# CliMA/ClimaOcean.jl

Measured on AMD Instinct MI355X. Metric: flux-kernel surface cells/s (update_state!: JRA55 interp + similarity-theory fluxes + net fluxes), higher is better.
Workload: dtype f64

## Files before the change

climaocean.jl_amd/csrc/coflux_abi.cpp:

```cpp
#include "coflux_ctx.hpp"

static thread_local std::string g_error;
static RcclApi g_rccl;

int cf_fail(cf_ctx* ctx, int code, const char* fmt, ...) {
    char buf[1024];
    va_list ap;
    va_start(ap, fmt);
    vsnprintf(buf, sizeof buf, fmt, ap);
    va_end(ap);
    g_error = buf;
    if (ctx) {
        std::lock_guard<std::mutex> lock(ctx->error_mutex);
        ctx->error = buf;
    }
    return code;
}

static int wait_for_halos(cf_ctx* ctx);
int cf_flush_deferred_prefetch(cf_ctx* ctx);

static bool roughness_ok(const cf_roughness& r, bool scalar) {
    if (scalar) {
        if (r.kind == CF_SCALAR_ROUGHNESS_CONSTANT) return r.constant_length > 0;
// ... 795 lines not shown
    if (ctx->deferred.valid && ctx->deferred.out.u == atmos->u) CHECK(cf_flush_deferred_prefetch(ctx));
    for (auto& p : ctx->prefetch) {
        if (!p.valid || p.key != atmos->u) continue;
        if (!p.on_main) HIP_TRY(ctx, hipStreamWaitEvent(ctx->stream, p.done, 0));
        prefetched = p.level1 == src->level1 && p.level2 == src->level2 && p.tf == src->time_fraction;
        p.valid = false;
    }
    const bool fuse = net_fluxes_fused(ctx);
    if (!prefetched) HIP_TRY(ctx, launch_interpolate(ctx->stream, ctx->launch, ctx->grid, src, w, atmos));
    if (rec) HIP_TRY(ctx, hipEventRecord(ev[1], ctx->stream));
    CHECK(wait_for_halos(ctx));
    const bool tail_lean = ctx->launch.d_lean_info && ctx->fast.specialization == SOLVER_OCEAN_LEAN && ctx->launch.solver == CF_SOLVER_TABLES;
    const bool tail_ly = ctx->fast.specialization == SOLVER_LY && ctx->launch.solver == CF_SOLVER_TABLES;
    const bool tail = fuse && !hold_tail_work && ctx->merged_prefetch == 2 && ctx->deferred.valid &&
                      interp_tile_fits(ctx, 40960) && ctx->deferred.out.u != atmos->u && (tail_lean || tail_ly);
    const bool ride = hold_tail_work && ocean_rider && fuse && tail_lean && !rec;
    HaloRider halo_rider{};
    const HaloRider* halo = nullptr;
    if (ctx->halo_request.valid) {
        ctx->halo_request.valid = false;
        if (tail && tail_lean && !ride && ctx->d_halo_counters && lean_halo_rides(ctx->launch, ctx->fast)) {
            HaloRider& H = halo_rider;
            H.M = ctx->peer;
            H.F = ctx->halo_request.F;
            H.counters = ctx->d_halo_counters;
            H.seq = ++ctx->peer_seq;
            ++ctx->halo_in_launch_count;
            for (int dir = 0; dir < 2; ++dir)
                if ((dir == 0 ? ctx->peer.south : ctx->peer.north) != nullptr) {
                    ctx->halo_expect_sent[dir] += (unsigned long long)H.F.n;
                    ctx->halo_expect_done[dir] += (unsigned long long)H.F.n;
                }
            for (int dir = 0; dir < 2; ++dir) {
                H.expect_sent[dir] = ctx->halo_expect_sent[dir];
                H.expect_done[dir] = ctx->halo_expect_done[dir];
            }
            H.status = ctx->d_peer_status;
            H.rows = ctx->halo_request.rows;
            H.blocks = 2 * H.F.n;
            H.chunk_south = ctx->launch.chunk_south;
            H.chunk_north = ctx->launch.chunk_north;
            H.wait_south = ctx->peer.south != nullptr;
            H.wait_north = ctx->peer.north != nullptr;
            halo = &halo_rider;
        } else {
            CHECK(cf_peer_halo_launch_now(ctx, &ctx->halo_request.F, ctx->halo_request.rows));
        }
    }
    if (ride) {
        HIP_TRY(ctx, make_ocean_rider(ctx->launch, ctx->dev, ctx->fast, ctx->grid, ocean, atmos, fluxes, ice, net, ctx->d_land_freshwater,
                                      ocean_rider));
    } else if (tail) {
        int rows = 4, blocks = 1;
        interpolate_grid(ctx->launch, ctx->grid, &rows, &blocks);
        static const int tail_cap = [] {
            const char* e = experiment_knob("COFLUX_TAIL_BLOCKS");
            return e ? std::max(1, std::atoi(e)) : 0;
        }();
        if (tail_cap > 0) blocks = std::min(blocks, tail_cap);
        static const int tail_pos = [] {
            const char* e = experiment_knob("COFLUX_TAIL_POS");
            return e ? std::atoi(e) : -1;
        }();
        if (tail_lean)
            HIP_TRY(ctx, launch_ao_fluxes_lean(ctx->stream, ctx->launch, ctx->dev, ctx->fast, ctx->grid, ocean, atmos, fluxes, ice, net,
                                               ctx->d_land_freshwater, &ctx->deferred.src, &ctx->deferred.w, &ctx->deferred.out, rows, blocks, tail_pos, halo));
        else
            HIP_TRY(ctx, launch_ly_fluxes_with_tail(ctx->stream, ctx->launch, ctx->dev, ctx->fast, ctx->grid, ocean, atmos, fluxes, ice, net,
                                                    ctx->d_land_freshwater, &ctx->deferred.src, &ctx->deferred.w, &ctx->deferred.out, rows, blocks));
        CHECK(deferred_went_out_on_main(ctx));
    } else
    HIP_TRY(ctx, launch_ao_fluxes(ctx->stream, ctx->launch, ctx->dev, ctx->fast, ctx->grid, ocean, atmos, fluxes,
                                  fuse ? ice : nullptr, fuse ? net : nullptr, ctx->d_land_freshwater));
    const bool merge = fuse && !hold_tail_work && ctx->merged_prefetch == 1 && ctx->deferred.valid && interp_tile_fits(ctx, 65536) &&
                       ctx->deferred.out.u != atmos->u;
    if (ctx->merged_prefetch == 0) CHECK(cf_flush_deferred_prefetch(ctx));
    if (rec) HIP_TRY(ctx, hipEventRecord(ev[2], ctx->stream));
    if (merge) {
        HIP_TRY(ctx, launch_interpolate_and_stress(ctx->stream, ctx->launch, ctx->dev, ctx->grid, &ctx->deferred.src, &ctx->deferred.w,
                                                   &ctx->deferred.out, ocean, fluxes, ice, net));
        CHECK(deferred_went_out_on_main(ctx));
    } else if (fuse && hold_tail_work) {
        if (stress_held) *stress_held = true;
    } else if (fuse)
        HIP_TRY(ctx, launch_net_stress(ctx->stream, ctx->dev, ctx->grid, ocean, fluxes, ice, net));
    else
        HIP_TRY(ctx, launch_net_fluxes(ctx->stream, ctx->dev, ctx->grid, ocean, atmos, fluxes, ice, w, net, ctx->d_land_freshwater));
    if (rec) {
        HIP_TRY(ctx, hipEventRecord(ev[3], ctx->stream));
        ++ctx->prof_count;
    }
    if (!hold_tail_work && ctx->merged_prefetch != 0 && ctx->deferred.valid && ctx->deferred.out.u != atmos->u) {
        HIP_TRY(ctx, launch_interpolate(ctx->stream, ctx->launch, ctx->grid, &ctx->deferred.src, &ctx->deferred.w, &ctx->deferred.out));
        CHECK(deferred_went_out_on_main(ctx));
    }
    return CF_OK;
}

int cf_update_state(cf_ctx* ctx, const cf_atmos_source* src, const cf_interp_weights* w,
                    const cf_ocean_surface* ocean, const cf_exchange_fields* atmos,
                    const cf_interface_fluxes* fluxes, const cf_sea_ice_fields* ice, const cf_net_ocean_fluxes* net) {
    return update_state_impl(ctx, src, w, ocean, atmos, fluxes, ice, net, false, nullptr);
}

int cf_profile_enable(cf_ctx* ctx, int max_records) {
    if (!ctx || max_records < 0) return fail(ctx, CF_ERR_INVALID, "cf_profile_enable: bad arguments");
    for (hipEvent_t e : ctx->prof_events) (void)hipEventDestroy(e);
// ... 513 lines not shown
```

climaocean.jl_amd/csrc/coflux_interp.hip:

```cpp
#include <hip/hip_runtime.h>

#include <algorithm>
#include <cstdlib>

#include "coflux_interp_cell.hpp"
#include "coflux_interp_tiles.hpp"
#include "coflux_kernel_types.hpp"
#include "coflux_kernels.h"

namespace coflux {

template <int ROWS>
__global__ __launch_bounds__(64 * IT_WAVES) void interpolate_kernel(SourceDesc S, WeightDesc Wt, GridDesc G,
                                                                     Exchange E, int cap) {
    interpolate_tiles<ROWS>(S, Wt, G, E, cap, (int)blockIdx.x, (int)gridDim.x);
}

struct StressArgs {
    const void* mask;
    const double* rtx;
    const double* rty;
    IceIn I;
    double* tau_x;
    double* tau_y;
// ... 86 lines not shown
    const int i = idx - jj * wx - G.ring, j = jj - G.ring;
    const size_t k = cell_index(G, i, j);
    const double fi = Wt.separable ? Wt.fi[i + G.hx] : Wt.fi[k];
    const double fj = Wt.separable ? Wt.fj[j + G.hy] : Wt.fj[k];
    const double xi = fi - floor(fi), eta = fj - floor(fj);
    const int i0 = (int)trunc(fi), ja = (int)trunc(fj);
    const int is0 = wrap_index(i0, ns_x), is1 = wrap_index(i0 + (fi > 0.0 ? 1 : (fi < 0.0 ? -1 : 0)), ns_x);
    const int j0 = min(max(ja, 0), ns_y - 1), j1 = min(max(ja + (fj > 0.0 ? 1 : (fj < 0.0 ? -1 : 0)), 0), ns_y - 1);
    const size_t g00 = (size_t)j0 * ns_x + is0, g10 = (size_t)j0 * ns_x + is1, g01 = (size_t)j1 * ns_x + is0, g11 = (size_t)j1 * ns_x + is1;
    const size_t plane = (size_t)ns_x * ns_y;
    const double w00 = (1.0 - xi) * (1.0 - eta), w01 = (1.0 - xi) * eta, w10 = xi * (1.0 - eta), w11 = xi * eta;
    auto value = [&](const float* d) {
        const float* a = d + (size_t)level1 * plane;
        const float* b = d + (size_t)level2 * plane;
        return bilinear(w00, w01, w10, w11, blend_levels(a[g00], b[g00], tf), blend_levels(a[g01], b[g01], tf),
                        blend_levels(a[g10], b[g10], tf), blend_levels(a[g11], b[g11], tf));
    };
    out[k] = value(friver) + (licalvf ? value(licalvf) : 0.0);
}

hipError_t launch_interpolate_land(hipStream_t st, const GridDesc& G, const cf_land_source* s, const cf_interp_weights* w, double* out) {
    const int n = (G.nx + 2 * G.ring) * (G.ny + 2 * G.ring);
    hipLaunchKernelGGL(interpolate_land_kernel, dim3((n + 255) / 256), dim3(256), 0, st, s->friver, s->licalvf, s->ns_x, s->ns_y,
                       s->level1, s->level2, s->time_fraction, make_weights(w), G, out);
    return hipGetLastError();
}

hipError_t launch_interpolate_background(hipStream_t st, const GridDesc& G, const cf_atmos_source* s,
                                         const cf_interp_weights* w, const cf_exchange_fields* e) {
    const int n = (G.nx + 2 * G.ring) * (G.ny + 2 * G.ring);
    hipLaunchKernelGGL(interpolate_gather_kernel, dim3((n + 255) / 256), dim3(256), 0, st, make_source(s), make_weights(w), G,
                       make_exchange(e));
    return hipGetLastError();
}

void interpolate_grid(const LaunchCfg& L, const GridDesc& G, int* rows_out, int* blocks_out) {
    const int wx = G.nx + 2 * G.ring, wy = G.ny + 2 * G.ring;
    const int tiles_x = (wx + 63) / 64;
    const long tiles4 = (long)tiles_x * ((wy + 3) / 4) * 256 / (L.cu_count > 0 ? L.cu_count : 256);
    const int rows = tiles4 >= 1200 ? 4 : (tiles4 >= 600 ? 2 : 1);
    const int ntiles = tiles_x * ((wy + rows - 1) / rows);
    int blocks = (ntiles + IT_WAVES - 1) / IT_WAVES;
    const int cus = L.cu_count > 0 ? L.cu_count : 256;
    if (blocks > 2 * cus && blocks <= 4 * cus) blocks = std::max(2 * cus, blocks * 25 / 32);
    static const int blocks_cap = [] {
        const char* cap = experiment_knob("COFLUX_INTERP_BLOCKS");
        return cap ? std::max(1, std::atoi(cap)) : 0;
    }();
    if (blocks_cap > 0) blocks = std::min(blocks, blocks_cap);
    *rows_out = rows;
    *blocks_out = blocks;
}

hipError_t launch_interpolate(hipStream_t st, const LaunchCfg& L, const GridDesc& G, const cf_atmos_source* s,
                              const cf_interp_weights* w, const cf_exchange_fields* e) {
    if (L.interp_cap == 0) return launch_interpolate_background(st, G, s, w, e);
    int rows = 4, blocks = 1;
    interpolate_grid(L, G, &rows, &blocks);
    const size_t lds = (size_t)IT_WAVES * CF_JRA55_NVARS * L.interp_cap * sizeof(double);
#define CF_LAUNCH_INTERP(ROWS_)                                                                                        \
    hipLaunchKernelGGL(interpolate_kernel<ROWS_>, dim3(blocks), dim3(64 * IT_WAVES), lds, st, make_source(s),          \
                       make_weights(w), G, make_exchange(e), L.interp_cap)
    if (rows == 4) CF_LAUNCH_INTERP(4);
    else if (rows == 2) CF_LAUNCH_INTERP(2);
    else CF_LAUNCH_INTERP(1);
#undef CF_LAUNCH_INTERP
    return hipGetLastError();
}

hipError_t launch_interpolate_and_stress(hipStream_t st, const LaunchCfg& L, const DevParams& P, const GridDesc& G,
                                         const cf_atmos_source* s, const cf_interp_weights* w, const cf_exchange_fields* e,
                                         const cf_ocean_surface* o, const cf_interface_fluxes* f, const cf_sea_ice_fields* ice,
                                         const cf_net_ocean_fluxes* n) {
    if (L.interp_cap == 0) return hipErrorInvalidValue;
    int rows = 4, blocks = 1;
    interpolate_grid(L, G, &rows, &blocks);
    const size_t lds = (size_t)IT_WAVES * CF_JRA55_NVARS * L.interp_cap * sizeof(double);
    StressArgs A{};
    A.mask = o->mask;
    A.rtx = f->x_momentum;
    A.rty = f->y_momentum;
    if (ice) A.I = IceIn{ice->concentration, ice->interface_heat, ice->salt_flux, ice->x_stress, ice->y_stress, nullptr};
    A.tau_x = n->u;
    A.tau_y = n->v;
    const int stress_blocks = (G.nx * G.ny + 255) / 256;
#define CF_LAUNCH_BOTH(ROWS_)                                                                                              \
    hipLaunchKernelGGL(interpolate_and_stress_kernel<ROWS_>, dim3(blocks + stress_blocks), dim3(64 * IT_WAVES), lds, st, \
                       make_source(s), make_weights(w), G, make_exchange(e), L.interp_cap, blocks, P, A)
    if (rows == 4) CF_LAUNCH_BOTH(4);
    else if (rows == 2) CF_LAUNCH_BOTH(2);
    else CF_LAUNCH_BOTH(1);
#undef CF_LAUNCH_BOTH
    return hipGetLastError();
}

}
```

climaocean.jl_amd/csrc/coflux_interp_tiles.hpp:

```cpp
#pragma once
#include <hip/hip_runtime.h>

#include <climits>

#include "coflux_interp_cell.hpp"
#include "coflux_kernel_types.hpp"

namespace coflux {

constexpr int IT_WAVES = 4;

template <bool MIN>
__device__ __forceinline__ int wave_reduce(int v) {
    auto op = [](int a, int b) { return MIN ? min(a, b) : max(a, b); };
    v = op(v, __builtin_amdgcn_update_dpp(v, v, 0xb1, 0xf, 0xf, false));
    v = op(v, __builtin_amdgcn_update_dpp(v, v, 0x4e, 0xf, 0xf, false));
    v = op(v, __builtin_amdgcn_update_dpp(v, v, 0x141, 0xf, 0xf, false));
    v = op(v, __builtin_amdgcn_update_dpp(v, v, 0x140, 0xf, 0xf, false));
    const int a = __builtin_amdgcn_readlane(v, 0), b = __builtin_amdgcn_readlane(v, 16);
    const int c = __builtin_amdgcn_readlane(v, 32), d = __builtin_amdgcn_readlane(v, 48);
    return op(op(a, b), op(c, d));
}
__device__ __forceinline__ int wave_min(int v) { return wave_reduce<true>(v); }
__device__ __forceinline__ int wave_max(int v) { return wave_reduce<false>(v); }

__device__ __forceinline__ void wave_lds_sync() {
    __builtin_amdgcn_fence(__ATOMIC_ACQ_REL, "wavefront");
    __builtin_amdgcn_wave_barrier();
}

template <int ROWS>
__device__ __forceinline__ void interpolate_tiles(const SourceDesc& S, const WeightDesc& Wt, const GridDesc& G, const Exchange& E, int cap,
                                                  int block, int nblocks) {
    extern __shared__ __attribute__((aligned(16))) char smem[];
    const int lane = threadIdx.x & 63, wave = threadIdx.x >> 6;
    double* tile = reinterpret_cast<double*>(smem) + (size_t)wave * CF_JRA55_NVARS * cap;

    const int wx = G.nx + 2 * G.ring, wy = G.ny + 2 * G.ring;
    const int tiles_x = (wx + 63) / 64, tiles_y = (wy + ROWS - 1) / ROWS;
    const int ntiles = tiles_x * tiles_y;
    const size_t plane = (size_t)S.ns_x * S.ns_y;
    const size_t off1 = (size_t)S.level1 * plane, off2 = (size_t)S.level2 * plane;
    const int half = S.ns_x / 2;
    const bool rotate = Wt.cos_rot != nullptr && Wt.sin_rot != nullptr;

    for (int t = block * IT_WAVES + wave; t < ntiles; t += nblocks * IT_WAVES) {
        const int ty = t / tiles_x, tx = t - ty * tiles_x;
        const int i = tx * 64 + lane - G.ring;
        const int ic = min(i, G.nx + G.ring - 1);

        int d0[ROWS], di[ROWS], j0[ROWS], j1[ROWS];
        double xi[ROWS], eta[ROWS];
        int lo = INT_MAX, hi = INT_MIN, jlo = INT_MAX, jhi = INT_MIN, ref = 0;
#pragma unroll
        for (int r = 0; r < ROWS; ++r) {
            const int jc = min(ty * ROWS + r - G.ring, G.ny + G.ring - 1);
            const size_t k = cell_index(G, ic, jc);
            const double fi = Wt.separable ? Wt.fi[ic + G.hx] : Wt.fi[k];
            const double fj = Wt.separable ? Wt.fj[jc + G.hy] : Wt.fj[k];
            const double ti = trunc(fi), tj = trunc(fj);
            xi[r] = fi - floor(fi);
            eta[r] = fj - floor(fj);
            const int i0 = (int)ti;
            di[r] = fi > 0.0 ? 1 : (fi < 0.0 ? -1 : 0);
            const int ja = (int)tj;
            const int jb = ja + (fj > 0.0 ? 1 : (fj < 0.0 ? -1 : 0));
            j0[r] = min(max(ja, 0), S.ns_y - 1);
            j1[r] = min(max(jb, 0), S.ns_y - 1);
            if (r == 0) ref = __shfl(i0, 0);
            d0[r] = wrap_index(i0 - ref + half, S.ns_x) - half;
            lo = min(lo, min(d0[r], d0[r] + di[r]));
            hi = max(hi, max(d0[r], d0[r] + di[r]));
            jlo = min(jlo, min(j0[r], j1[r]));
            jhi = max(jhi, max(j0[r], j1[r]));
        }
        lo = wave_min(lo);
        hi = wave_max(hi);
        jlo = wave_min(jlo);
        jhi = wave_max(jhi);
        const int W = hi - lo + 1, H = jhi - jlo + 1, WH = W * H;
        const bool fits = WH <= cap && W <= S.ns_x;

        if (fits) {
            const float inv_W = 1.0f / (float)W;
            for (int rem = lane; rem < WH; rem += 64) {
                const int y = (int)(((float)rem + 0.5f) * inv_W);
// ... 59 lines not shown
```

climaocean.jl_amd/csrc/coflux_kernels.h:

```cpp
#pragma once
#include <hip/hip_runtime.h>

#include <cstdlib>

#include "coflux_device.hpp"

namespace coflux {

inline const char* experiment_knob(const char* name) {
    static const bool enabled = [] {
        const char* e = std::getenv("COFLUX_EXPERIMENTS");
        return e != nullptr && e[0] == '1';
    }();
    return enabled ? std::getenv(name) : nullptr;
}


struct LoopParams;
struct IceParams;
struct HaloRider;

struct LaunchCfg {
    int solver;
    int interp_cap;
    int ao_chunk;
    int cu_count;
    const double* d_tables;
    const DevParams* d_params;
    uint8_t* d_trip;
    const int* d_chunk_begins;
    int n_chunks;
    int chunk_south, chunk_north;
    const uint32_t* d_wet_pos;
    uint32_t* d_lean_sorted;
    const int* d_lean_info;
    int lean_hints;
    int certified;
    int latency_layout;
};

bool lean_line_applies(const LaunchCfg& L, const LoopParams& C, bool coare);

bool lean_certified_applies(const LaunchCfg& L, const LoopParams& C);

hipError_t launch_interpolate(hipStream_t st, const LaunchCfg& L, const GridDesc& G, const cf_atmos_source* s,
                              const cf_interp_weights* w, const cf_exchange_fields* e);
hipError_t launch_ao_fluxes(hipStream_t st, const LaunchCfg& L, const DevParams& P, const LoopParams& C,
                            const GridDesc& G, const cf_ocean_surface* o, const cf_exchange_fields* e,
                            const cf_interface_fluxes* f, const cf_sea_ice_fields* ice = nullptr,
                            const cf_net_ocean_fluxes* net = nullptr, const double* land = nullptr);
hipError_t launch_net_stress(hipStream_t st, const DevParams& P, const GridDesc& G, const cf_ocean_surface* o,
                             const cf_interface_fluxes* f, const cf_sea_ice_fields* ice, const cf_net_ocean_fluxes* n);
hipError_t build_wet_lists(hipStream_t st, const DevParams* d_params, const GridDesc& G, const void* mask, int nchunks,
                           const int* d_begins, uint32_t* d_wet_pos, uint8_t* d_trip, int* d_scratch, int* overflow_out);
hipError_t build_lean_lists(hipStream_t st, int nchunks, const uint32_t* d_wet_pos, const int* d_begins, uint32_t* d_sorted, int* d_info);
hipError_t launch_ly_fluxes_with_tail(hipStream_t st, const LaunchCfg& L, const DevParams& P, const LoopParams& C, const GridDesc& G,
                                      const cf_ocean_surface* o, const cf_exchange_fields* e, const cf_interface_fluxes* f,
                                      const cf_sea_ice_fields* ice, const cf_net_ocean_fluxes* net, const double* land,
                                      const cf_atmos_source* next_src, const cf_interp_weights* w, const cf_exchange_fields* next_out,
                                      int tail_rows, int tail_blocks);
hipError_t launch_ao_fluxes_lean(hipStream_t st, const LaunchCfg& L, const DevParams& P, const LoopParams& C, const GridDesc& G,
                                 const cf_ocean_surface* o, const cf_exchange_fields* e, const cf_interface_fluxes* f,
                                 const cf_sea_ice_fields* ice = nullptr, const cf_net_ocean_fluxes* net = nullptr, const double* land = nullptr,
                                 const cf_atmos_source* next_src = nullptr, const cf_interp_weights* w = nullptr,
                                 const cf_exchange_fields* next_out = nullptr, int tail_rows = 0, int tail_blocks = 0, int tail_pos = -1,
                                 const HaloRider* halo = nullptr);
bool lean_halo_rides(const LaunchCfg& L, const LoopParams& C);
size_t wet_list_capacity(int ncells);
int wet_list_stride();
hipError_t launch_ao_fluxes_libm(hipStream_t st, const DevParams& P, const GridDesc& G, const cf_ocean_surface* o,
                                 const cf_exchange_fields* e, const cf_interface_fluxes* f);
hipError_t launch_net_fluxes(hipStream_t st, const DevParams& P, const GridDesc& G, const cf_ocean_surface* o,
                             const cf_exchange_fields* e, const cf_interface_fluxes* f, const cf_sea_ice_fields* ice,
                             const cf_interp_weights* w, const cf_net_ocean_fluxes* n, const double* land = nullptr);
hipError_t launch_interpolate_land(hipStream_t st, const GridDesc& G, const cf_land_source* s, const cf_interp_weights* w, double* out);
hipError_t launch_salinity_restoring(hipStream_t st, const DevParams& P, const GridDesc& G, const void* mask, double vp,
                                     const double* target, const double* S, double* out);
void interpolate_grid(const LaunchCfg& L, const GridDesc& G, int* rows_out, int* blocks_out);
hipError_t launch_interpolate_and_stress(hipStream_t st, const LaunchCfg& L, const DevParams& P, const GridDesc& G,
                                         const cf_atmos_source* s, const cf_interp_weights* w, const cf_exchange_fields* e,
                                         const cf_ocean_surface* o, const cf_interface_fluxes* f, const cf_sea_ice_fields* ice,
                                         const cf_net_ocean_fluxes* n);
hipError_t launch_interpolate_background(hipStream_t st, const GridDesc& G, const cf_atmos_source* s,
                                         const cf_interp_weights* w, const cf_exchange_fields* e);
struct OceanRider {
    alignas(16) unsigned char args[1536];
    int n_chunks = 0;
    bool coare = false, valid = false;
};
hipError_t make_ocean_rider(const LaunchCfg& L, const DevParams& P, const LoopParams& C, const GridDesc& G, const cf_ocean_surface* o,
                            const cf_exchange_fields* e, const cf_interface_fluxes* f, const cf_sea_ice_fields* ice,
                            const cf_net_ocean_fluxes* net, const double* land, OceanRider* out);
struct AiTail {
    const OceanRider* ocean = nullptr;
    const cf_atmos_source* next_src = nullptr;
    const cf_interp_weights* w = nullptr;
    const cf_exchange_fields* next_out = nullptr;
    int interp_rows = 0, interp_blocks = 0;
    const DevParams* d_ocean_params = nullptr;
    const cf_ocean_surface* stress_ocean = nullptr;
    const cf_interface_fluxes* stress_fluxes = nullptr;
    const cf_sea_ice_fields* stress_ice = nullptr;
    const cf_net_ocean_fluxes* stress_net = nullptr;
};
hipError_t launch_ai_fluxes(hipStream_t st, const LaunchCfg& L, const DevParams& P, const LoopParams& C, const IceParams& I,
                            const GridDesc& G, const cf_sea_ice_state* ice, const cf_ocean_surface* o,
                            const cf_exchange_fields* e, const cf_interface_fluxes* f, const double* d_tables,
                            const DevParams* d_params, uint8_t* d_trip, const AiTail* tail = nullptr, const NetIceOut* net_ice = nullptr);
constexpr int AO_PLAN_TAIL = -2;
hipError_t build_chunk_table(hipStream_t st, const DevParams* d_params, const GridDesc& G, const void* mask, int cu_count,
                             int wet_per_chunk, int* d_sums, int* d_begins, int* d_meta, int* wet_per_chunk_out,
                             int* nchunks_out);
int chunk_table_capacity(int ncells);
int chunk_sums_capacity(int ncells);
hipError_t launch_net_sea_ice_fluxes(hipStream_t st, const DevParams& P, const GridDesc& G, const void* mask,
                                     const cf_sea_ice_state* ice, double albedo, double emissivity, double eps_sigma,
                                     double T_offset, const cf_exchange_fields* e, const cf_interface_fluxes* f,
                                     const double* frazil, const double* interface_heat, const cf_net_sea_ice_fluxes* out);
hipError_t launch_sea_ice_albedo(hipStream_t st, const cf_sea_ice_albedo_params& A, const GridDesc& G, const double* hi,
                                 const double* hs, const double* Ts, double* out);
hipError_t launch_sea_ice_ocean_fluxes(hipStream_t st, const DevParams& P, const cf_ice_ocean_params& Q, const GridDesc& G,
                                       const cf_ocean_surface* o, const double* conc, const double* tx, const double* ty,
                                       const cf_ice_ocean_fluxes* out);
constexpr int SALINITY_PARTIAL_BLOCKS = 512;
hipError_t launch_salinity_partial_sums(hipStream_t st, const DevParams& P, const GridDesc& G, const double* flux,
                                        const double* additional, const double* area, const void* mask, double* partial,
                                        int nblocks, double* sums);
hipError_t launch_salinity_subtract(hipStream_t st, const GridDesc& G, double* flux, const double* sums, double* mean_out);
hipError_t launch_debug_eval(hipStream_t st, const LaunchCfg& L, int fn, int n, const double* x, double* y);
struct PeerMailbox;
struct PeerFields;
// ... 14 lines not shown
```

climaocean.jl_amd/csrc/coflux_lean_kernel.hpp:

```cpp
#pragma once
#include <hip/hip_runtime.h>

#include "coflux_halo_device.hpp"
#include "coflux_interp_tiles.hpp"
#include "coflux_lean.hpp"
#include "coflux_certified.hpp"
#include "coflux_solver_shared.hpp"

#ifndef CF_LEAN_WAVES
#define CF_LEAN_WAVES 3
#endif
#ifndef CF_LEAN_PREFETCH
#define CF_LEAN_PREFETCH 0
#endif

#ifndef LEAN_STAMP
#define LEAN_STAMP(q) do { } while (0)
#define LEAN_STAMP_SET(q, v) do { } while (0)
#endif

namespace coflux {

struct LeanArgs {
    LoopParams L;
    GridDesc G;
    OceanIn O;
    Exchange E;
    FluxOut F;
    const double* g_tab;
    const DevParams* g_params;
    uint32_t* sorted;
    const int* info;
    const int* chunk_begins;
    double z_surface;
    long long mask_kind;
    double T_offset;
    unsigned long long wx_reciprocal;
    long long sort_enabled;
    IceIn I;
    NetOut N;
    SourceDesc S;
    WeightDesc Wt;
    Exchange E_next;
    long long n_chunks;
    long long tail_blocks, tail_rows, tail_cap;
    long long tail_pos;
    HaloRider H;
};
typedef const LeanArgs __attribute__((address_space(4)))* LeanArgsPtr;

hipError_t launch_ao_lean_line(hipStream_t st, bool coare, bool fuse, bool tail, bool halo, int blocks, const LeanArgs& A);

__device__ __forceinline__ LeanArgsPtr opaque(LeanArgsPtr p) {
    asm volatile("" : "+s"(p));
    return p;
}

__device__ __forceinline__ unsigned lean_mix(unsigned idx) { return (idx * 0x9e3779b1u) ^ ((idx * 0x85ebca6bu) >> 15); }
__device__ __forceinline__ unsigned lean_sum(unsigned idx) { return idx * 0xc2b2ae35u + 0x27d4eb2fu; }

constexpr int LEAN_LIST_OFFSET = TABLE_BYTES;
constexpr int LEAN_OFFSET_BITS = 24;
constexpr unsigned LEAN_OFFSET_MASK = (1u << LEAN_OFFSET_BITS) - 1u;
static_assert((long)AO_CHUNK * AO_WET_COST < (1L << LEAN_OFFSET_BITS), "a chunk's range must fit the offset bits");
template <int BLOCK>
struct LeanGeom {
    static_assert(BLOCK == AO_BLOCK, "one workgroup geometry: 256 threads, three workgroups per CU (the 768-thread one-per-CU geometry of rounds 2-5 measured 3 % slower and was retired in round 6)");
    static constexpr int CHUNK = AO_CHUNK;
    static constexpr int WAVES = BLOCK / 64;
    static constexpr int HIST_OFFSET = LEAN_LIST_OFFSET + CHUNK * 4;
    static constexpr int CURSOR_OFFSET = HIST_OFFSET + AO_BINS * 4;
    static constexpr int COUNTERS_OFFSET = CURSOR_OFFSET + AO_BINS * 4;
    static constexpr int WAVEHASH_OFFSET = COUNTERS_OFFSET + 16;
    static constexpr int PARAMS_OFFSET = WAVEHASH_OFFSET + WAVES * 8;
    static constexpr int LDS_BYTES = PARAMS_OFFSET + (int)sizeof(DevParams);
    static_assert(PARAMS_OFFSET % 16 == 0 && LEAN_LIST_OFFSET % 1024 == 0 && (CHUNK * 4) % 1024 == 0, "LDS-DMA pieces");
};
static_assert(LeanGeom<AO_BLOCK>::LDS_BYTES <= 53760, "three narrow lean solver workgroups must fit the CU's 160 KB of LDS");
#ifndef CF_SKIP_LDS_ASSERT
static_assert(CF_LEAN_WAVES <= 3 || LeanGeom<AO_BLOCK>::LDS_BYTES <= 40960, "four narrow lean workgroups per CU: 160 KB / 4 in 1280-byte granules");
#endif

template <bool FUSE>
__device__ __forceinline__ void lean_zero_cell(const LoopParams& L, double T_offset, const GridDesc& G, LeanArgsPtr K, size_t k, int i, int j) {
    CellFluxes Z{};
    Z.Ts_ocean = -T_offset;
    Z.iterations = L.fixed ? L.maxiter : 0;
    const FluxOut F = kread(&K->F);
    store_fluxes(F, k, Z);
    if constexpr (FUSE) {
        if (i >= 0 && i < G.nx && j >= 0 && j < G.ny) {
            const NetOut N = kread(&K->N);
            store_net_cell(N, k, NetCell{});
        }
    }
}

#ifndef CF_CERT_NET_SALT
#define CF_CERT_NET_SALT 1
#endif
template <bool COARE, bool FUSE, bool TAIL = false, bool CERT = false, bool LINE = false, bool HALO = false>
__device__ __forceinline__ void ao_lean_body(LeanArgsPtr K_in, int chunk_in) {
    constexpr int BLOCK = AO_BLOCK;
    using Geo = LeanGeom<BLOCK>;
    constexpr int CHUNK = Geo::CHUNK;
    LeanArgsPtr K = opaque(K_in);
    int chunk = chunk_in;
    bool wait_south = false, wait_north = false;
    if constexpr (HALO) {
        static_assert(TAIL && !CERT, "the halo riders belong to the stepping loop's exact-path launch");
        const int nh = K->H.blocks;
        if (chunk < nh) {
            extern __shared__ __attribute__((aligned(16))) char smem_h[];
            const int nf = K->H.F.n, dir = chunk / nf, f = chunk - dir * nf;
            const PeerMailbox M = kread(&K->H.M);
            const GridDesc Gh = kread(&K->G);
            peer_halo_rider(M, K->H.F.ptr[f], f, dir, K->H.rows, K->H.seq, K->H.counters, K->H.expect_sent[dir], K->H.status, Gh, BLOCK,
                            reinterpret_cast<int*>(smem_h));
            return;
        }
        chunk -= nh;
    }
    if constexpr (TAIL) {
        static_assert(BLOCK == 64 * IT_WAVES, "a tail workgroup is an interpolation workgroup");
        const int nb = (int)K->tail_blocks, ipos = (int)K->tail_pos;
        if (chunk >= ipos && chunk < ipos + nb) {
            const SourceDesc S = kread(&K->S);
            const WeightDesc Wt = kread(&K->Wt);
            const GridDesc Gt = kread(&K->G);
            const Exchange En = kread(&K->E_next);
            const int b = chunk - ipos, cap = (int)K->tail_cap, rows = (int)K->tail_rows;
            if (rows == 4) interpolate_tiles<4>(S, Wt, Gt, En, cap, b, nb);
            else if (rows == 2) interpolate_tiles<2>(S, Wt, Gt, En, cap, b, nb);
            else interpolate_tiles<1>(S, Wt, Gt, En, cap, b, nb);
            return;
        }
        if (chunk >= ipos) chunk -= nb;
    }
    if constexpr (HALO) {
        const int cs = K->H.chunk_south, cn = K->H.chunk_north, nc = (int)K->n_chunks;
        if (K->H.blocks > 0) {
            if (cs <= cn) {
                const int inner = cn - cs;
                chunk = chunk < inner ? cs + chunk : (chunk - inner < cs ? chunk - inner : cn + (chunk - inner - cs));
            }
            wait_south = K->H.wait_south != 0 && chunk < cs;
            wait_north = K->H.wait_north != 0 && chunk >= cn && chunk < nc;
        }
    }
    const LoopParams L = kread(&K->L);
    const GridDesc G = kread(&K->G);
    const double* __restrict__ g_tab = K->g_tab;
    const DevParams* __restrict__ g_params = K->g_params;
    const void* mask = K->O.mask;
    extern __shared__ __attribute__((aligned(16))) char smem[];
    double* tab = reinterpret_cast<double*>(smem);
    unsigned* list = reinterpret_cast<unsigned*>(smem + LEAN_LIST_OFFSET);
    int* hist = reinterpret_cast<int*>(smem + Geo::HIST_OFFSET);
    int* cursor = reinterpret_cast<int*>(smem + Geo::CURSOR_OFFSET);
    int* counters = reinterpret_cast<int*>(smem + Geo::COUNTERS_OFFSET);
    unsigned* wavehash = reinterpret_cast<unsigned*>(smem + Geo::WAVEHASH_OFFSET);
    DevParams* lp = reinterpret_cast<DevParams*>(smem + Geo::PARAMS_OFFSET);
    const int tid = threadIdx.x, lane = tid & 63, wave = tid >> 6;
    LEAN_STAMP(0);
    const int wx = G.nx + 2 * G.ring;
    const unsigned wx_rcp = (unsigned)K->wx_reciprocal;
    const bool use_static = K->sorted != nullptr;
    unsigned long long stamp_iter = 0, stamp_batches = 0, stamp_trips = 0;
    static_assert(sizeof(DevParams) % 16 == 0 && sizeof(DevParams) <= 1024, "the parameter block is one LDS-DMA piece");
    if (tid < (int)(sizeof(DevParams) / 16))
        __builtin_amdgcn_global_load_lds((const __attribute__((address_space(1))) void*)(reinterpret_cast<const char*>(g_params) + lane * 16),
                                         (__attribute__((address_space(3))) void*)(smem + Geo::PARAMS_OFFSET), 16, 0, 0);
    static_assert(TABLE_BYTES % 1024 == 0, "the table stage copies whole 1 KB pieces");
    {
        const char* gb = reinterpret_cast<const char*>(g_tab);
        constexpr int PIECES = TABLE_BYTES / 1024, WAVES = Geo::WAVES;
#pragma unroll
        for (int r = 0; r < (PIECES + WAVES - 1) / WAVES; ++r) {
            const int c = wave + r * WAVES;
            if (c < PIECES)
                __builtin_amdgcn_global_load_lds((const __attribute__((address_space(1))) void*)(gb + c * 1024 + lane * 16),
                                                 (__attribute__((address_space(3))) void*)(smem + c * 1024), 16, 0, 0);
        }
    }
    if (use_static) {
        const char* gl = reinterpret_cast<const char*>(K->sorted + (size_t)chunk * CHUNK);
        constexpr int PIECES = CHUNK * 4 / 1024, WAVES = Geo::WAVES;
// ... 393 lines not shown
```

climaocean.jl_amd/csrc/coflux_solver_lean.hip:

```cpp
#include <hip/hip_runtime.h>

#include <algorithm>
#include <cstdlib>
#include <cstring>


namespace coflux {

#ifdef CF_LEAN_STAMPS
__device__ unsigned long long g_lean_stamp[4096 * 8];
#define LEAN_STAMP(q) do { if (lane == 0) g_lean_stamp[((size_t)blockIdx.x * (blockDim.x >> 6) + wave) * 8 + (q)] = __builtin_readcyclecounter(); } while (0)
#define LEAN_STAMP_SET(q, v) do { if (lane == 0) g_lean_stamp[((size_t)blockIdx.x * (blockDim.x >> 6) + wave) * 8 + (q)] = (v); } while (0)
extern "C" int cf_debug_phase_read(unsigned long long* out, int n) {
    (void)hipDeviceSynchronize();
    (void)hipMemcpyFromSymbol(out, HIP_SYMBOL(g_lean_stamp), sizeof(unsigned long long) * n);
    return 0;
}
#else
#define LEAN_STAMP(q) do { } while (0)
#define LEAN_STAMP_SET(q, v) do { } while (0)
#endif
}

#include "coflux_lean_kernel.hpp"

namespace coflux {

template <bool COARE, bool FUSE, bool TAIL = false, bool CERT = false>
__global__ __launch_bounds__(AO_BLOCK, CF_LEAN_WAVES) void ao_lean_kernel(LeanArgs unused_by_name) {
    ao_lean_body<COARE, FUSE, TAIL, CERT>((LeanArgsPtr)__builtin_amdgcn_kernarg_segment_ptr(), (int)blockIdx.x);
}

template <bool COARE>
__global__ __launch_bounds__(AO_BLOCK, CF_LEAN_WAVES) void ao_lean_halo_kernel(LeanArgs unused_by_name) {
    ao_lean_body<COARE, true, true, false, false, true>((LeanArgsPtr)__builtin_amdgcn_kernarg_segment_ptr(), (int)blockIdx.x);
}

__global__ __launch_bounds__(256) void lean_list_build_kernel(const uint32_t* __restrict__ wet_pos, const int* __restrict__ begins, int stride,
                                                              uint32_t* __restrict__ sorted, int* __restrict__ info) {
    __shared__ unsigned sx[4], sy[4];
    __shared__ int sn[4];
    const int chunk = blockIdx.x, lane = threadIdx.x & 63, wave = threadIdx.x >> 6;
    const int begin = begins[chunk];
    unsigned hx = 0, hy = 0;
    int n = 0;
    for (int e = threadIdx.x; e < stride; e += 256) {
        const uint32_t idx = wet_pos[(size_t)chunk * stride + e];
        const bool listed = idx != 0xffffffffu;
        sorted[(size_t)chunk * stride + e] = listed ? idx - (uint32_t)begin : LEAN_OFFSET_MASK;
        if (listed) {
            hx ^= lean_mix(idx);
            hy += lean_sum(idx);
            ++n;
        }
    }
    for (int d = 32; d; d >>= 1) {
        hx ^= (unsigned)__shfl_xor((int)hx, d);
        hy += (unsigned)__shfl_xor((int)hy, d);
        n += __shfl_xor(n, d);
    }
    if (lane == 0) {
        sx[wave] = hx;
        sy[wave] = hy;
        sn[wave] = n;
    }
    __syncthreads();
    if (threadIdx.x == 0) {
        info[chunk * 4] = sn[0] + sn[1] + sn[2] + sn[3];
        info[chunk * 4 + 1] = (int)(sx[0] ^ sx[1] ^ sx[2] ^ sx[3]);
        info[chunk * 4 + 2] = (int)(sy[0] + sy[1] + sy[2] + sy[3]);
        info[chunk * 4 + 3] = 0;
    }
}

hipError_t build_lean_lists(hipStream_t st, int nchunks, const uint32_t* d_wet_pos, const int* d_begins, uint32_t* d_sorted, int* d_info) {
    hipLaunchKernelGGL(lean_list_build_kernel, dim3(nchunks), dim3(256), 0, st, d_wet_pos, d_begins, AO_CHUNK, d_sorted, d_info);
    return hipGetLastError();
}

bool lean_certified_applies(const LaunchCfg& L, const LoopParams& C) {
    return L.certified && C.specialization == SOLVER_OCEAN_LEAN && !C.fixed && L.lean_hints == 0 &&
           C.cert_max_evals > 2 && C.tol >= 1e-9 && C.maxiter >= 40;
}

bool lean_halo_rides(const LaunchCfg& L, const LoopParams& C) {
    return C.specialization == SOLVER_OCEAN_LEAN && L.solver == CF_SOLVER_TABLES && !lean_certified_applies(L, C);
}

bool lean_line_applies(const LaunchCfg& L, const LoopParams& C, bool coare) {
    if (L.latency_layout == 0 || C.specialization != SOLVER_OCEAN_LEAN || C.beta_gust == 0.0) return false;
    if (lean_certified_applies(L, C)) return false;
    return L.latency_layout == 2 || (coare && L.cu_count > 0 && L.n_chunks <= 2 * L.cu_count);
}

static hipError_t fill_lean_args(const LaunchCfg& L, const DevParams& P, const LoopParams& C, const GridDesc& G, const cf_ocean_surface* o,
                                 const cf_exchange_fields* e, const cf_interface_fluxes* f, const cf_sea_ice_fields* ice,
                                 const cf_net_ocean_fluxes* net, const double* land, LeanArgs& A) {
    if (!L.d_chunk_begins || L.n_chunks <= 0 || !L.d_lean_info) return hipErrorInvalidValue;
    A.L = C;
    A.G = G;
    A.O = make_ocean(o);
    A.E = make_exchange(e);
    A.F = make_fluxes(f);
    A.g_tab = L.d_tables;
    A.g_params = L.d_params;
    A.sorted = L.d_wet_pos ? L.d_lean_sorted : nullptr;
    A.info = L.d_lean_info;
    A.chunk_begins = L.d_chunk_begins;
    A.z_surface = P.z_surface;
    A.mask_kind = P.mask_kind;
    A.T_offset = P.T_offset;
    A.wx_reciprocal = row_reciprocal(G.nx + 2 * G.ring);
    A.sort_enabled = L.lean_hints;
    if (L.lean_hints > 1) {
        static const int windows = [] {
            const char* e = experiment_knob("COFLUX_SORT_WINDOWS");
            return e ? std::max(1, std::min(8, std::atoi(e))) : 0;
        }();
        if (windows > 0) A.sort_enabled = windows;
    }
    if (net) {
        if (ice) A.I = IceIn{ice->concentration, ice->interface_heat, ice->salt_flux, ice->x_stress, ice->y_stress, nullptr};
        A.I.land = land;
        A.N = NetOut{net->u, net->v, net->T, net->S, net->shortwave_surface_flux, net->upwelling_longwave, net->downwelling_longwave,
                     net->downwelling_shortwave};
    }
    return hipSuccess;
}

hipError_t make_ocean_rider(const LaunchCfg& L, const DevParams& P, const LoopParams& C, const GridDesc& G, const cf_ocean_surface* o,
                            const cf_exchange_fields* e, const cf_interface_fluxes* f, const cf_sea_ice_fields* ice,
                            const cf_net_ocean_fluxes* net, const double* land, OceanRider* out) {
    static_assert(sizeof(LeanArgs) <= sizeof(out->args), "OceanRider::args holds a LeanArgs");
    if (!out || !net) return hipErrorInvalidValue;
    LeanArgs A{};
    if (hipError_t err = fill_lean_args(L, P, C, G, o, e, f, ice, net, land, A)) return err;
    memcpy(out->args, &A, sizeof(A));
    out->n_chunks = L.n_chunks;
    out->coare = P.similarity_form == CF_SIMILARITY_COARE_LOGARITHMIC;
    out->valid = true;
    return hipSuccess;
}

hipError_t launch_ao_fluxes_lean(hipStream_t st, const LaunchCfg& L, const DevParams& P, const LoopParams& C, const GridDesc& G,
                                 const cf_ocean_surface* o, const cf_exchange_fields* e, const cf_interface_fluxes* f,
                                 const cf_sea_ice_fields* ice, const cf_net_ocean_fluxes* net, const double* land,
                                 const cf_atmos_source* next_src, const cf_interp_weights* w, const cf_exchange_fields* next_out,
                                 int tail_rows, int tail_blocks, int tail_pos, const HaloRider* halo) {
    LeanArgs A{};
    if (hipError_t err = fill_lean_args(L, P, C, G, o, e, f, ice, net, land, A)) return err;
    const bool coare = P.similarity_form == CF_SIMILARITY_COARE_LOGARITHMIC;
    const bool cert = lean_certified_applies(L, C);
    const bool tail = next_out != nullptr;
    int blocks = L.n_chunks;
    if (tail) {
        if (!net || !next_src || !w || L.interp_cap <= 0 || tail_blocks <= 0) return hipErrorInvalidValue;
        const size_t tile_lds = (size_t)IT_WAVES * CF_JRA55_NVARS * L.interp_cap * sizeof(double);
        if (tile_lds > (size_t)LeanGeom<AO_BLOCK>::LDS_BYTES) return hipErrorInvalidValue;
        A.S = make_source(next_src);
        A.Wt = make_weights(w);
        A.E_next = make_exchange(next_out);
        A.n_chunks = L.n_chunks;
        A.tail_blocks = tail_blocks;
        A.tail_rows = tail_rows;
        A.tail_cap = L.interp_cap;
        A.tail_pos = tail_pos < 0 || tail_pos > L.n_chunks ? L.n_chunks : tail_pos;
        blocks += tail_blocks;
    }
    const bool riders = halo != nullptr && halo->blocks > 0;
    if (riders) {
        if (!tail || !lean_halo_rides(L, C) || halo->F.n < 1 || halo->blocks != 2 * halo->F.n) return hipErrorInvalidValue;
        A.H = *halo;
        blocks += halo->blocks;
    }
    if (lean_line_applies(L, C, coare)) return launch_ao_lean_line(st, coare, net != nullptr, tail, riders, blocks, A);
    if (riders) {
        if (coare) hipLaunchKernelGGL((ao_lean_halo_kernel<true>), dim3(blocks), dim3(AO_BLOCK), LeanGeom<AO_BLOCK>::LDS_BYTES, st, A);
        else hipLaunchKernelGGL((ao_lean_halo_kernel<false>), dim3(blocks), dim3(AO_BLOCK), LeanGeom<AO_BLOCK>::LDS_BYTES, st, A);
        return hipGetLastError();
    }
#define CF_LEAN_LAUNCH(COARE_, FUSE_, TAIL_, CERT_) \
    hipLaunchKernelGGL((ao_lean_kernel<COARE_, FUSE_, TAIL_, CERT_>), dim3(blocks), dim3(AO_BLOCK), LeanGeom<AO_BLOCK>::LDS_BYTES, st, A)
#define CF_LEAN_PICK(FUSE_, TAIL_)                                                       \
    do {                                                                                 \
        if (cert) {                                                                      \
            if (coare) CF_LEAN_LAUNCH(true, FUSE_, TAIL_, true); else CF_LEAN_LAUNCH(false, FUSE_, TAIL_, true);   \
        } else {                                                                         \
            if (coare) CF_LEAN_LAUNCH(true, FUSE_, TAIL_, false); else CF_LEAN_LAUNCH(false, FUSE_, TAIL_, false); \
        }                                                                                \
    } while (0)
    if (tail) CF_LEAN_PICK(true, true);
    else if (net) CF_LEAN_PICK(true, false);
    else CF_LEAN_PICK(false, false);
#undef CF_LEAN_PICK
#undef CF_LEAN_LAUNCH
    return hipGetLastError();
}

}
```

Baseline: 9.893 billion.

## Software-pipeline tail interpolation tiles and shrink tail block count

Adds a pipelined variant of the tile interpolation used by the lean flux kernel's interpolation tail: each wave prefetches the next tile's source footprint into registers while it computes and stores the current tile. Corner indices are packed into 32-bit words to save registers. The tail grid is also resized so each wave handles about two tiles, which gives the pipeline something to overlap. This is meant to hide global load latency in the tail, at the cost of more register pressure and fewer blocks. It also extends the debug timestamp instrumentation.

```diff
diff --git a/climaocean.jl_amd/csrc/coflux_abi.cpp b/climaocean.jl_amd/csrc/coflux_abi.cpp
--- a/climaocean.jl_amd/csrc/coflux_abi.cpp
+++ b/climaocean.jl_amd/csrc/coflux_abi.cpp
@@ -871,7 +871,10 @@
                                       ocean_rider));
     } else if (tail) {
         int rows = 4, blocks = 1;
-        interpolate_grid(ctx->launch, ctx->grid, &rows, &blocks);
+        const bool coare = ctx->dev.similarity_form == CF_SIMILARITY_COARE_LOGARITHMIC;
+        if (tail_lean && lean_tail_pipelined(ctx->launch, ctx->fast, coare, halo != nullptr, &ctx->deferred.src))
+            interpolate_tail_grid(ctx->launch, ctx->grid, &rows, &blocks);
+        else interpolate_grid(ctx->launch, ctx->grid, &rows, &blocks);
         static const int tail_cap = [] {
             const char* e = experiment_knob("COFLUX_TAIL_BLOCKS");
             return e ? std::max(1, std::atoi(e)) : 0;
diff --git a/climaocean.jl_amd/csrc/coflux_interp.hip b/climaocean.jl_amd/csrc/coflux_interp.hip
--- a/climaocean.jl_amd/csrc/coflux_interp.hip
+++ b/climaocean.jl_amd/csrc/coflux_interp.hip
@@ -162,6 +162,28 @@
     *blocks_out = blocks;
 }
 
+bool interpolate_tail_pipelined() {
+    static const bool on = [] {
+        const char* e = experiment_knob("COFLUX_TAIL_PIPE");
+        return !(e && e[0] == '0');
+    }();
+    return on;
+}
+
+constexpr int IT_TAIL_TILES = 2;
+void interpolate_tail_grid(const LaunchCfg& L, const GridDesc& G, int* rows_out, int* blocks_out) {
+    interpolate_grid(L, G, rows_out, blocks_out);
+    static const int tiles_per_wave = [] {
+        const char* e = experiment_knob("COFLUX_TAIL_TILES");
+        return e ? std::max(1, std::atoi(e)) : IT_TAIL_TILES;
+    }();
+    const int cus = L.cu_count > 0 ? L.cu_count : 256;
+    const int wx = G.nx + 2 * G.ring, wy = G.ny + 2 * G.ring;
+    const int ntiles = ((wx + 63) / 64) * ((wy + *rows_out - 1) / *rows_out);
+    if (*blocks_out > 2 * cus)
+        *blocks_out = std::max(1, (ntiles + IT_WAVES * tiles_per_wave - 1) / (IT_WAVES * tiles_per_wave));
+}
+
 hipError_t launch_interpolate(hipStream_t st, const LaunchCfg& L, const GridDesc& G, const cf_atmos_source* s,
                               const cf_interp_weights* w, const cf_exchange_fields* e) {
     if (L.interp_cap == 0) return launch_interpolate_background(st, G, s, w, e);
diff --git a/climaocean.jl_amd/csrc/coflux_interp_tiles.hpp b/climaocean.jl_amd/csrc/coflux_interp_tiles.hpp
--- a/climaocean.jl_amd/csrc/coflux_interp_tiles.hpp
+++ b/climaocean.jl_amd/csrc/coflux_interp_tiles.hpp
@@ -30,8 +30,242 @@
 }
 
 template <int ROWS>
+struct TileIndex {
+    int ty, i;
+    unsigned c[ROWS];
+    double xi[ROWS], eta[ROWS];
+    int lo, jlo, ref, W, WH;
+    bool fits;
+};
+
+constexpr int IT_PACKED_NODES = 16383;
+__host__ __device__ __forceinline__ bool interpolate_tiles_fit_packing(int ns_x, int ns_y) {
+    return ns_x <= IT_PACKED_NODES && ns_y <= IT_PACKED_NODES;
+}
+__device__ __forceinline__ unsigned corner_word(int d0, int di, int j0, int j1) {
+    return ((unsigned)(d0 + 8192) << 18) | ((unsigned)j0 << 4) | ((unsigned)(j1 - j0 + 1) << 2) | (unsigned)(di + 1);
+}
+struct Corners {
+    int d0, di, j0, j1;
+};
+__device__ __forceinline__ Corners corners_of(unsigned c) {
+    Corners k;
+    k.di = (int)(c & 3u) - 1;
+    k.j0 = (int)((c >> 4) & 0x3fffu);
+    k.j1 = k.j0 + (int)((c >> 2) & 3u) - 1;
+    k.d0 = (int)(c >> 18) - 8192;
+    return k;
+}
+
+struct TileJob {
+    int tiles_x, ntiles, half;
+    size_t off1, off2;
+    bool rotate;
+};
+
+template <int ROWS>
+__device__ __forceinline__ TileJob tile_job(const SourceDesc& S, const WeightDesc& Wt, const GridDesc& G) {
+    TileJob J;
+    const int wx = G.nx + 2 * G.ring, wy = G.ny + 2 * G.ring;
+    J.tiles_x = (wx + 63) / 64;
+    J.ntiles = J.tiles_x * ((wy + ROWS - 1) / ROWS);
+    const size_t plane = (size_t)S.ns_x * S.ns_y;
+    J.off1 = (size_t)S.level1 * plane;
+    J.off2 = (size_t)S.level2 * plane;
+    J.half = S.ns_x / 2;
+    J.rotate = Wt.cos_rot != nullptr && Wt.sin_rot != nullptr;
+    return J;
+}
+
+template <int ROWS>
+__device__ __forceinline__ TileIndex<ROWS> tile_index(const SourceDesc& S, const WeightDesc& Wt, const GridDesc& G, const TileJob& J,
+                                                      int cap, int t, int lane) {
+    TileIndex<ROWS> T;
+    T.ty = t / J.tiles_x;
+    const int tx = t - T.ty * J.tiles_x;
+    T.i = tx * 64 + lane - G.ring;
+    const int ic = min(T.i, G.nx + G.ring - 1);
+    int lo = INT_MAX, hi = INT_MIN, jlo = INT_MAX, jhi = INT_MIN, ref = 0;
+#pragma unroll
+    for (int r = 0; r < ROWS; ++r) {
+        const int jc = min(T.ty * ROWS + r - G.ring, G.ny + G.ring - 1);
+        const size_t k = cell_index(G, ic, jc);
+        const double fi = Wt.separable ? Wt.fi[ic + G.hx] : Wt.fi[k];
+        const double fj = Wt.separable ? Wt.fj[jc + G.hy] : Wt.fj[k];
+        const double ti = trunc(fi), tj = trunc(fj);
+        T.xi[r] = fi - floor(fi);
+        T.eta[r] = fj - floor(fj);
+        const int i0 = (int)ti;
+        const int di = fi > 0.0 ? 1 : (fi < 0.0 ? -1 : 0);
+        const int ja = (int)tj;
+        const int jb = ja + (fj > 0.0 ? 1 : (fj < 0.0 ? -1 : 0));
+        const int j0 = min(max(ja, 0), S.ns_y - 1);
+        const int j1 = min(max(jb, 0), S.ns_y - 1);
+        if (r == 0) ref = __shfl(i0, 0);
+        const int d0 = wrap_index(i0 - ref + J.half, S.ns_x) - J.half;
+        T.c[r] = corner_word(d0, di, j0, j1);
+        lo = min(lo, min(d0, d0 + di));
+        hi = max(hi, max(d0, d0 + di));
+        jlo = min(jlo, min(j0, j1));
+        jhi = max(jhi, max(j0, j1));
+    }
+    lo = wave_min(lo);
+    hi = wave_max(hi);
+    jlo = wave_min(jlo);
+    jhi = wave_max(jhi);
+    T.lo = lo;
+    T.jlo = jlo;
+    T.ref = ref;
+    T.W = hi - lo + 1;
+    T.WH = T.W * (jhi - jlo + 1);
+    T.fits = T.WH <= cap && T.W <= S.ns_x;
+    return T;
+}
+
+template <int ROWS>
+__device__ __forceinline__ size_t footprint_offset(const SourceDesc& S, const TileIndex<ROWS>& T, float inv_W, int rem) {
+    const int y = (int)(((float)rem + 0.5f) * inv_W);
+    const int x = rem - y * T.W;
+    return (size_t)(T.jlo + y) * S.ns_x + wrap_index(T.ref + T.lo + x, S.ns_x);
+}
+
+template <int ROWS>
+__device__ __forceinline__ void stage_footprint(const SourceDesc& S, const TileJob& J, const TileIndex<ROWS>& T, double* tile, int cap,
+                                                int lane, int from) {
+    if (!T.fits) return;
+    const float inv_W = 1.0f / (float)T.W;
+    for (int rem = from + lane; rem < T.WH; rem += 64) {
+        const size_t off = footprint_offset(S, T, inv_W, rem);
+#pragma unroll
+        for (int v = 0; v < CF_JRA55_NVARS; ++v)
+            tile[v * cap + rem] = blend_levels(S.data[v][J.off1 + off], S.data[v][J.off2 + off], S.tf);
+    }
+}
+
+constexpr int IT_HELD_PASSES = 1;
+struct FootprintRaw {
+    float a[IT_HELD_PASSES][CF_JRA55_NVARS], b[IT_HELD_PASSES][CF_JRA55_NVARS];
+};
+
+template <int ROWS>
+__device__ __forceinline__ void request_footprint(const SourceDesc& S, const TileJob& J, const TileIndex<ROWS>& T, int lane, FootprintRaw& R) {
+    if (!T.fits) return;
+    const float inv_W = 1.0f / (float)T.W;
+#pragma unroll
+    for (int p = 0; p < IT_HELD_PASSES; ++p) {
+        if (64 * p >= T.WH) break;
+        const size_t off = footprint_offset(S, T, inv_W, min(lane + 64 * p, T.WH - 1));
+#pragma unroll
+        for (int v = 0; v < CF_JRA55_NVARS; ++v) {
+            R.a[p][v] = S.data[v][J.off1 + off];
+            R.b[p][v] = S.data[v][J.off2 + off];
+        }
+    }
+}
+
+template <int ROWS>
+__device__ __forceinline__ void blend_footprint(const SourceDesc& S, const TileJob& J, const TileIndex<ROWS>& T, const FootprintRaw& R,
+                                                double* tile, int cap, int lane) {
+    if (!T.fits) return;
+#pragma unroll
+    for (int p = 0; p < IT_HELD_PASSES; ++p) {
+        const int rem = lane + 64 * p;
+        if (rem < T.WH) {
+#pragma unroll
+            for (int v = 0; v < CF_JRA55_NVARS; ++v) tile[v * cap + rem] = blend_levels(R.a[p][v], R.b[p][v], S.tf);
+        }
+    }
+    stage_footprint(S, J, T, tile, cap, lane, 64 * IT_HELD_PASSES);
+}
+
+template <int ROWS>
+__device__ __forceinline__ void interpolate_store(const SourceDesc& S, const WeightDesc& Wt, const GridDesc& G, const Exchange& E,
+                                                  const TileJob& J, const TileIndex<ROWS>& T, const double* tile, int cap) {
+#pragma unroll
+    for (int r = 0; r < ROWS; ++r) {
+        const int j = T.ty * ROWS + r - G.ring;
+        const double w00 = (1.0 - T.xi[r]) * (1.0 - T.eta[r]), w01 = (1.0 - T.xi[r]) * T.eta[r];
+        const double w10 = T.xi[r] * (1.0 - T.eta[r]), w11 = T.xi[r] * T.eta[r];
+        const Corners c = corners_of(T.c[r]);
+        double val[CF_JRA55_NVARS];
+        if (T.fits) {
+            const int o00 = (c.j0 - T.jlo) * T.W + (c.d0 - T.lo), o01 = (c.j1 - T.jlo) * T.W + (c.d0 - T.lo);
+#pragma unroll
+            for (int v = 0; v < CF_JRA55_NVARS; ++v) {
+                const double* p = tile + v * cap;
+                val[v] = bilinear(w00, w01, w10, w11, p[o00], p[o01], p[o00 + c.di], p[o01 + c.di]);
+            }
+        } else {
+            const int is0 = wrap_index(T.ref + c.d0, S.ns_x), is1 = wrap_index(T.ref + c.d0 + c.di, S.ns_x);
+            const size_t g00 = (size_t)c.j0 * S.ns_x + is0, g10 = (size_t)c.j0 * S.ns_x + is1;
+            const size_t g01 = (size_t)c.j1 * S.ns_x + is0, g11 = (size_t)c.j1 * S.ns_x + is1;
+#pragma unroll
+            for (int v = 0; v < CF_JRA55_NVARS; ++v) {
+                const float* a = S.data[v] + J.off1;
+                const float* b = S.data[v] + J.off2;
+                val[v] = bilinear(w00, w01, w10, w11, blend_levels(a[g00], b[g00], S.tf), blend_levels(a[g01], b[g01], S.tf),
+                                  blend_levels(a[g10], b[g10], S.tf), blend_levels(a[g11], b[g11], S.tf));
+            }
+        }
+        if (T.i < G.nx + G.ring && j < G.ny + G.ring) {
+            const size_t k = cell_index(G, T.i, j);
+            double ua = val[CF_JRA55_UAS], va = val[CF_JRA55_VAS];
+            if (J.rotate) {
+                const double cs = Wt.cos_rot[k], sn = Wt.sin_rot[k];
+                const double ui = ua * cs + va * sn;
+                va = -ua * sn + va * cs;
+                ua = ui;
+            }
+            E.u[k] = ua;
+            E.v[k] = va;
+            E.T[k] = val[CF_JRA55_TAS];
+            E.p[k] = val[CF_JRA55_PSL];
+            E.q[k] = val[CF_JRA55_HUSS];
+            E.Qs[k] = val[CF_JRA55_RSDS];
+            E.Ql[k] = val[CF_JRA55_RLDS];
+            E.Mp[k] = val[CF_JRA55_PRRA] + val[CF_JRA55_PRSN];
+        }
+    }
+}
+
+template <int ROWS>
+__device__ __forceinline__ void interpolate_tiles_pipelined(const SourceDesc& S, const WeightDesc& Wt, const GridDesc& G, const Exchange& E,
+                                                            int cap, int block, int nblocks) {
+    extern __shared__ __attribute__((aligned(16))) char smem[];
+    const int lane = threadIdx.x & 63, wave = threadIdx.x >> 6;
+    double* tile = reinterpret_cast<double*>(smem) + (size_t)wave * CF_JRA55_NVARS * cap;
+    const TileJob J = tile_job<ROWS>(S, Wt, G);
+    const int stride = nblocks * IT_WAVES;
+    int t = block * IT_WAVES + wave;
+    if (t >= J.ntiles) return;
+    TileIndex<ROWS> cur = tile_index<ROWS>(S, Wt, G, J, cap, t, lane);
+    FootprintRaw raw;
+    request_footprint(S, J, cur, lane, raw);
+    for (;;) {
+        blend_footprint(S, J, cur, raw, tile, cap, lane);
+        wave_lds_sync();
+        const int tn = t + stride;
+        const bool more = tn < J.ntiles;
+        TileIndex<ROWS> nxt;
+        if (more) {
+            nxt = tile_index<ROWS>(S, Wt, G, J, cap, tn, lane);
+            request_footprint(S, J, nxt, lane, raw);
+        }
+        interpolate_store(S, Wt, G, E, J, cur, tile, cap);
+        wave_lds_sync();
+        if (!more) break;
+        cur = nxt;
+        t = tn;
+    }
+}
+
+template <int ROWS, bool PIPE = false>
 __device__ __forceinline__ void interpolate_tiles(const SourceDesc& S, const WeightDesc& Wt, const GridDesc& G, const Exchange& E, int cap,
                                                   int block, int nblocks) {
+    if constexpr (PIPE) {
+        interpolate_tiles_pipelined<ROWS>(S, Wt, G, E, cap, block, nblocks);
+        return;
+    }
     extern __shared__ __attribute__((aligned(16))) char smem[];
     const int lane = threadIdx.x & 63, wave = threadIdx.x >> 6;
     double* tile = reinterpret_cast<double*>(smem) + (size_t)wave * CF_JRA55_NVARS * cap;
diff --git a/climaocean.jl_amd/csrc/coflux_kernels.h b/climaocean.jl_amd/csrc/coflux_kernels.h
--- a/climaocean.jl_amd/csrc/coflux_kernels.h
+++ b/climaocean.jl_amd/csrc/coflux_kernels.h
@@ -65,6 +65,7 @@
                                  const cf_atmos_source* next_src = nullptr, const cf_interp_weights* w = nullptr,
                                  const cf_exchange_fields* next_out = nullptr, int tail_rows = 0, int tail_blocks = 0, int tail_pos = -1,
                                  const HaloRider* halo = nullptr);
+bool lean_tail_pipelined(const LaunchCfg& L, const LoopParams& C, bool coare, bool halo, const cf_atmos_source* s);
 bool lean_halo_rides(const LaunchCfg& L, const LoopParams& C);
 size_t wet_list_capacity(int ncells);
 int wet_list_stride();
@@ -77,6 +78,8 @@
 hipError_t launch_salinity_restoring(hipStream_t st, const DevParams& P, const GridDesc& G, const void* mask, double vp,
                                      const double* target, const double* S, double* out);
 void interpolate_grid(const LaunchCfg& L, const GridDesc& G, int* rows_out, int* blocks_out);
+bool interpolate_tail_pipelined();
+void interpolate_tail_grid(const LaunchCfg& L, const GridDesc& G, int* rows_out, int* blocks_out);
 hipError_t launch_interpolate_and_stress(hipStream_t st, const LaunchCfg& L, const DevParams& P, const GridDesc& G,
                                          const cf_atmos_source* s, const cf_interp_weights* w, const cf_exchange_fields* e,
                                          const cf_ocean_surface* o, const cf_interface_fluxes* f, const cf_sea_ice_fields* ice,
diff --git a/climaocean.jl_amd/csrc/coflux_lean_kernel.hpp b/climaocean.jl_amd/csrc/coflux_lean_kernel.hpp
--- a/climaocean.jl_amd/csrc/coflux_lean_kernel.hpp
+++ b/climaocean.jl_amd/csrc/coflux_lean_kernel.hpp
@@ -45,6 +45,7 @@
     long long n_chunks;
     long long tail_blocks, tail_rows, tail_cap;
     long long tail_pos;
+    long long tail_pipe;
     HaloRider H;
 };
 typedef const LeanArgs __attribute__((address_space(4)))* LeanArgsPtr;
@@ -130,9 +131,24 @@
             const GridDesc Gt = kread(&K->G);
             const Exchange En = kread(&K->E_next);
             const int b = chunk - ipos, cap = (int)K->tail_cap, rows = (int)K->tail_rows;
-            if (rows == 4) interpolate_tiles<4>(S, Wt, Gt, En, cap, b, nb);
-            else if (rows == 2) interpolate_tiles<2>(S, Wt, Gt, En, cap, b, nb);
-            else interpolate_tiles<1>(S, Wt, Gt, En, cap, b, nb);
+            [[maybe_unused]] const int lane = threadIdx.x & 63, wave = threadIdx.x >> 6;
+            LEAN_STAMP(0);
+            constexpr bool CAN_PIPE = !COARE && !LINE && !HALO;
+            bool pipe = false;
+            if constexpr (CAN_PIPE) pipe = K->tail_pipe != 0;
+            if (pipe) {
+                if constexpr (CAN_PIPE) {
+                    if (rows == 4) interpolate_tiles<4, true>(S, Wt, Gt, En, cap, b, nb);
+                    else if (rows == 2) interpolate_tiles<2, true>(S, Wt, Gt, En, cap, b, nb);
+                    else interpolate_tiles<1, true>(S, Wt, Gt, En, cap, b, nb);
+                }
+            } else {
+                if (rows == 4) interpolate_tiles<4>(S, Wt, Gt, En, cap, b, nb);
+                else if (rows == 2) interpolate_tiles<2>(S, Wt, Gt, En, cap, b, nb);
+                else interpolate_tiles<1>(S, Wt, Gt, En, cap, b, nb);
+            }
+            LEAN_STAMP(5);
+            LEAN_STAMP_SET(7, LEAN_TAIL_MARK);
             return;
         }
         if (chunk >= ipos) chunk -= nb;
diff --git a/climaocean.jl_amd/csrc/coflux_solver_lean.hip b/climaocean.jl_amd/csrc/coflux_solver_lean.hip
--- a/climaocean.jl_amd/csrc/coflux_solver_lean.hip
+++ b/climaocean.jl_amd/csrc/coflux_solver_lean.hip
@@ -8,12 +8,27 @@
 namespace coflux {
 
 #ifdef CF_LEAN_STAMPS
-__device__ unsigned long long g_lean_stamp[4096 * 8];
-#define LEAN_STAMP(q) do { if (lane == 0) g_lean_stamp[((size_t)blockIdx.x * (blockDim.x >> 6) + wave) * 8 + (q)] = __builtin_readcyclecounter(); } while (0)
-#define LEAN_STAMP_SET(q, v) do { if (lane == 0) g_lean_stamp[((size_t)blockIdx.x * (blockDim.x >> 6) + wave) * 8 + (q)] = (v); } while (0)
+constexpr size_t LEAN_STAMP_WAVES = 8192;
+constexpr unsigned long long LEAN_TAIL_MARK = 1ull << 48;
+__device__ unsigned long long g_lean_stamp[LEAN_STAMP_WAVES * 8];
+__device__ unsigned long long g_lean_rt[LEAN_STAMP_WAVES * 2];
+#define LEAN_STAMP_WAVE ((size_t)blockIdx.x * (blockDim.x >> 6) + wave)
+#define LEAN_STAMP(q)                                                                                              \
+    do {                                                                                                           \
+        if (lane == 0 && LEAN_STAMP_WAVE < LEAN_STAMP_WAVES) {                                                     \
+            g_lean_stamp[LEAN_STAMP_WAVE * 8 + (q)] = __builtin_readcyclecounter();                                \
+            if ((q) == 0 || (q) == 5) g_lean_rt[LEAN_STAMP_WAVE * 2 + ((q) == 5)] = __builtin_amdgcn_s_memrealtime(); \
+        }                                                                                                          \
+    } while (0)
+#define LEAN_STAMP_SET(q, v) do { if (lane == 0 && LEAN_STAMP_WAVE < LEAN_STAMP_WAVES) g_lean_stamp[LEAN_STAMP_WAVE * 8 + (q)] = (v); } while (0)
 extern "C" int cf_debug_phase_read(unsigned long long* out, int n) {
     (void)hipDeviceSynchronize();
-    (void)hipMemcpyFromSymbol(out, HIP_SYMBOL(g_lean_stamp), sizeof(unsigned long long) * n);
+    (void)hipMemcpyFromSymbol(out, HIP_SYMBOL(g_lean_stamp), sizeof(unsigned long long) * std::min<size_t>(n, LEAN_STAMP_WAVES * 8));
+    return 0;
+}
+extern "C" int cf_debug_phase_read_realtime(unsigned long long* out, int n) {
+    (void)hipDeviceSynchronize();
+    (void)hipMemcpyFromSymbol(out, HIP_SYMBOL(g_lean_rt), sizeof(unsigned long long) * std::min<size_t>(n, LEAN_STAMP_WAVES * 2));
     return 0;
 }
 #else
@@ -85,6 +100,11 @@
 
 bool lean_halo_rides(const LaunchCfg& L, const LoopParams& C) {
     return C.specialization == SOLVER_OCEAN_LEAN && L.solver == CF_SOLVER_TABLES && !lean_certified_applies(L, C);
+}
+
+bool lean_tail_pipelined(const LaunchCfg& L, const LoopParams& C, bool coare, bool halo, const cf_atmos_source* s) {
+    return interpolate_tail_pipelined() && !coare && !halo && !lean_line_applies(L, C, coare) && s != nullptr &&
+           interpolate_tiles_fit_packing(s->ns_x, s->ns_y);
 }
 
 bool lean_line_applies(const LaunchCfg& L, const LoopParams& C, bool coare) {
@@ -168,6 +188,7 @@
         blocks += tail_blocks;
     }
     const bool riders = halo != nullptr && halo->blocks > 0;
+    if (tail) A.tail_pipe = lean_tail_pipelined(L, C, coare, riders, next_src) ? 1 : 0;
     if (riders) {
         if (!tail || !lean_halo_rides(L, C) || halo->F.n < 1 || halo->blocks != 2 * halo->F.n) return hipErrorInvalidValue;
         A.H = *halo;
```

Result: slower. 9.225 billion (-6.8%).
